# facebook/facebook360_dep

Measured on AMD Instinct MI355X. Metric: depth Mpix/s per GPU (full pyramid, 16-cam 2048^2 rig); % HBM-read roofline, higher is better.
Workload: dtype f32+f64; 1 GPU; BASELINE config 3: 16-camera 2048x2048 synthetic rig, 8-frame sequence, full 10-level pyramid per frame, per-level temporal filter (+-2 frames); the same sequence for every --gpus N (block partition, 8 frame(s) on this rank); rig=cfg2, cameras=16, frames=8, temporal_filter=True, halo_transport=local, parallelism=frames x1

## Files before the change

facebook360_dep_amd/csrc/derp_capi.hip:

```cpp
#include <hip/hip_runtime.h>

#include <algorithm>
#include <cfloat>
#include <cmath>
#include <cstdarg>
#include <cstdio>
#include <cstdlib>
#include <cstring>
#include <map>
#include <memory>
#include <string>
#include <vector>

#include <rocprim/device/device_radix_sort.hpp>

#include "../../include/derp_hip.h"
#include "derp_host.h"
#include "derp_kernels.h"
#include "derp_mesh.h"
#include "derp_points.h"
#include "derp_render.h"
#include "derp_geometric.h"
#include "derp_sweep.h"

// ... 360 lines not shown
  return 0;
}

int build_warp(derp_ctx* c, int dst0, int nd) {
  const int L = c->cur;
  Span sp(c, ST_PROJ_WARP, L);
  {
    const size_t n = (size_t)c->LW[L] * c->LH[L];
    ALLOC(c, c->rayDir, 3 * n * c->D * sizeof(double));
    ALLOC(c, c->behind, n * c->D * sizeof(unsigned));
  }
  LevelView V = make_view(c, ST_PROJ_WARP, dst0, nd);
  hipLaunchKernelGGL(k_proj_warp, grid2d(V.W + 2 * kPadW, V.H + 2 * kPadW, c->S, kBlk2d), kBlk2d, 0, c->stream, V,
                     c->projWarp.as<float2>());
  KCHECK(c);
  hipLaunchKernelGGL(k_pixel_rays, grid2d(V.W, V.H, nd, kBlk2d), kBlk2d, 0, c->stream, V, c->rayDir.as<double>(),
                     c->behind.as<unsigned>());
  KCHECK(c);
  c->w.colorTablesCleanLevel = -1;
  if (batch_needs_inverse_warps(c, dst0, nd)) {
    hipLaunchKernelGGL(k_proj_warp_inv, grid2d(V.W, V.H, nd, kBlk2d), kBlk2d, 0, c->stream, V, c->projWarpInv.as<float2>());
    KCHECK(c);
  }
  return 0;
}

int build_color_tables(derp_ctx* c, int dst0, int nd) {
  const int L = c->cur;
  LevelView V = make_view(c, ST_REPROJECT, dst0, nd);
  Span sp(c, ST_REPROJECT, L);
  const dim3 grid((V.W + kRbTile - 1) / kRbTile, (V.H + kRbTile - 1) / kRbTile, nd * (c->S - 1));
  ALLOC(c, c->w.tileSeen, (size_t)grid.x * grid.y * grid.z);
  const int skipBlank = c->w.colorTablesCleanLevel == L && nd == c->D && !c->noBlankSkip;
  hipLaunchKernelGGL(k_reproject_bias, grid, dim3(256), 0, c->stream, V, c->projWarpInv.as<float2>(),
                     c->w.projColor.as<ushort4>(), c->w.projBias.as<ushort4>(), c->w.projColorT.as<ushort4>(),
                     c->w.tileSeen.as<uint8_t>(), skipBlank);
  KCHECK(c);
  c->w.colorTablesCleanLevel = nd == c->D ? L : -1;
  return 0;
}

int tiles_of(int W, int H, int& tilesX) {
  constexpr int B = kTileBlock;
  tilesX = ((W + 15) / 16 + B - 1) / B * B;
  const int tilesY = ((H + 15) / 16 + B - 1) / B * B;
  return tilesX * tilesY * (256 / kCostBlock);
}
constexpr size_t kCostLdsPerSrc = (size_t)kCostBlock * sizeof(SsdPair);
struct CostGrid {
  int blocks, bands, perBlock;
};
constexpr int kCostMaxBands = 4, kCostMaxTilesPerBlock = 4;
int cost_grid_blocks(int tiles, int bands, int perBlock) {
  const int items = (tiles + perBlock - 1) / perBlock, unit = 8 * bands;
  return (items + unit - 1) / unit * unit;
}
CostGrid cost_grid(const derp_ctx* c, int tiles, int tilesX, bool spread) {
  const auto pow2_floor = [](int v, int cap) {
    int p = 1;
    while (p * 2 <= std::min(v, cap)) {
      p *= 2;
    }
    return p;
  };
  CostGrid g;
  g.perBlock = c->costTilesPerBlock > 0 ? pow2_floor(c->costTilesPerBlock, kCostMaxTilesPerBlock) : 1;
  const int rowOfSquares = tilesX * (256 / kCostBlock) * kTileBlock;
// ... 117 lines not shown
  }
  for (int d = 0; d < c->D; ++d) {
    if (c->dst2srcH[d] != d) {
      return fail(c, "mismatch handling needs destinations in rig order (dst %d maps to src %d)", d, c->dst2srcH[d]);
    }
  }
  Span sp(c, ST_MISMATCH, L);
  c->randomRanThisLevel = false;
  LevelView V = make_view(c, ST_MISMATCH, 0, c->D);
  const size_t n = (size_t)V.W * V.H;
  hipLaunchKernelGGL(k_mismatch, dim3((V.W + 15) / 16, (V.H + 15) / 16, c->D), dim3(256), 256 * sizeof(float) * c->S,
                     c->stream, V, c->w.dispRes.as<float>(), c->w.mismatchMask.as<uint8_t>());
  KCHECK(c);
  HIPCHK(c, hipMemcpyAsync(c->w.disparity.p, c->w.dispRes.p, n * c->D * sizeof(float), hipMemcpyDeviceToDevice, c->stream));
  return 0;
}

int bilateral_radius(int level) {
  const float scale = std::pow(0.9f, level);
  return (int)std::max(std::ceil(5 * scale), float(1));
}

size_t bilateral_lds_bytes(int radius) {
  const size_t side = 16 + 2 * (size_t)radius;
  const size_t t = ((side + 15) & ~(size_t)15) * side;
  return t * 4 * sizeof(float) + ((t + 3) & ~(size_t)3);
}

constexpr size_t kBilateralMaxLds = 64 * 1024 - 256;

bool bilateral_fast_tap_ok(float sigma, float w0, float w1, float w2) {
  const float denom = 2.0f * (sigma * sigma);
  return w1 == 1.0f && w2 == 1.0f && w0 >= 0.0f && std::isfinite(w0) && denom > 0.0f && std::isfinite(denom);
}

void launch_joint_bilateral_u16_tiled(derp_ctx* c, dim3 grid, const float* image, const void* guide, const uint8_t* mask,
                                      int W, int H, int radius, float sigma, float w0, float w1, float w2, float* out,
                                      size_t planeStride, size_t guideStride, const int* guideIndex) {
  const bool fast = bilateral_fast_tap_ok(sigma, w0, w1, w2) && bilateral_lds_bytes(radius) + 256 <= kBilateralMaxLds;
  const auto kernel = fast ? k_joint_bilateral<true, true> : k_joint_bilateral<true, false>;
  hipLaunchKernelGGL(kernel, grid, dim3(256), bilateral_lds_bytes(radius), c->stream, image, guide, mask, W, H, radius, sigma,
                     w0, w1, w2, out, planeStride, guideStride, guideIndex);
}

int run_bilateral(derp_ctx* c) {
  const int L = c->cur;
  Span sp(c, ST_BILATERAL, L);
  c->randomRanThisLevel = false;
  const int W = c->LW[L], H = c->LH[L];
  const size_t n = (size_t)W * H;
  const int radius = bilateral_radius(L);
  launch_joint_bilateral_u16_tiled(c, dim3((W + 15) / 16, (H + 15) / 16, c->D), c->w.disparity.as<float>(),
                                   (const void*)c->frame().color[L].as<ushort4>(), c->w.maskAnd.as<uint8_t>(), W, H, radius,
                                   0.005f, 0.5f, 1.0f, 1.0f, c->w.tmpF.as<float>(), n, n, c->dst2src.as<int>());
  KCHECK(c);
  std::swap(c->w.disparity, c->w.tmpF);
  return 0;
}

int run_median(derp_ctx* c, bool fuseMaskFov, float* levelOut = nullptr) {
  const int L = c->cur;
  Span sp(c, ST_MEDIAN, L);
  c->randomRanThisLevel = false;
  const int W = c->LW[L], H = c->LH[L];
  const size_t n = (size_t)W * H;
  hipLaunchKernelGGL(k_masked_median, grid2d(W, H, c->D, kBlk2d), kBlk2d, 0, c->stream, c->w.disparity.as<float>(),
// ... 281 lines not shown
    rc = fail(c, "work lane: hipEventRecord failed");
  }
  lane_swap(c, i);
  c->activeLane = -1;
  c->cur = -1;
  return rc;
}

int temporal_launch(derp_ctx* c, const void* const* guides, const float* const* images, const uint8_t* const* masks, int n,
                    int centre, int W, int H, int planes, float sigma, int radius, float w0, float w1, float w2,
                    float* out, const int* dst2src) {
  if (n < 1 || centre < 0 || centre >= n) {
    return fail(c, "temporal window must hold at least the centre frame");
  }
  if (n > kMaxTemporalFrames) {
    ALLOC(c, c->temporalCarry, (size_t)planes * W * H * sizeof(float2));
  }
  for (int t0 = 0; t0 < n; t0 += kMaxTemporalFrames) {
    TemporalFrames F;
    F.n = std::min(kMaxTemporalFrames, n - t0);
    for (int t = 0; t < F.n; ++t) {
      F.guides[t] = reinterpret_cast<const ushort4*>(guides[t0 + t]);
      F.images[t] = images[t0 + t];
      F.masks[t] = masks[t0 + t];
    }
    F.refGuide = reinterpret_cast<const ushort4*>(guides[centre]);
    F.refImage = images[centre];
    F.refMask = masks[centre];
    F.carry = n > kMaxTemporalFrames ? c->temporalCarry.as<float2>() : nullptr;
    F.first = t0 == 0;
    F.last = t0 + F.n >= n;
    const size_t lds = 2 * ((((size_t)(32 + 2 * radius) * (8 + 2 * radius) * 9) + 15) & ~(size_t)15);
    if (radius >= 0 && lds <= 48 * 1024 && !c->noTemporalTile) {
      hipLaunchKernelGGL(k_temporal_tiled, grid2d(W, H, planes, kBlk2d), kBlk2d, lds, c->stream, F, W, H, sigma, radius, w0,
                         w1, w2, out, dst2src);
    } else {
      hipLaunchKernelGGL(k_temporal, grid2d(W, H, planes, kBlk2d), kBlk2d, 0, c->stream, F, W, H, sigma, radius, w0, w1, w2,
                         out, dst2src);
    }
    KCHECK(c);
  }
  return 0;
}

}

extern "C" {

void derp_options_default(derp_options* o) {
  o->min_depth_m = 0.5f;
  o->max_depth_m = 1e4f;
  o->var_noise_floor = 4e-5f;
  o->var_high_thresh = 1e-3f;
  o->random_proposals = 2;
  o->ping_pong_iterations = 1;
  o->mismatches_start_level = -1;
  o->do_bilateral_filter = 1;
  o->do_median_filter = 1;
  o->use_foreground_masks = 0;
  o->partial_coverage = 0;
  o->rebuild_warp_tables = 1;
}

int derp_create(derp_ctx** out, int device, const derp_camera_desc* src, int n_src, const derp_camera_desc* dst,
                int n_dst) {
  if (!out) {
    return 1;
  }
// ... 4 lines not shown
  if (n_src <= 0 || n_dst <= 0) {
    return create_fail("no source / destination cameras!");
  }
  hipDeviceProp_t prop;
  TRY(open_device(device, "the depth path", &prop));
  c->device = device;
  if (prop.maxSharedMemoryPerMultiProcessor > 0) {
    c->ldsPerCu = prop.maxSharedMemoryPerMultiProcessor;
  }
  if (const char* e = getenv("DERP_XCD_ROTATE")) {
    c->xcdRotate = atoi(e);
  }
  if (const char* e = getenv("DERP_XCD_BANDS")) {
    c->xcdBands = atoi(e);
  }
  if (const char* e = getenv("DERP_COST_TILES_PER_BLOCK")) {
    c->costTilesPerBlock = atoi(e);
  }
  c->noMemo = getenv("DERP_NO_MEMO") != nullptr;
  if (const char* e = getenv("DERP_BRUTE_RUN")) {
    c->bruteRun = atoi(e);
  }
  if (const char* e = getenv("DERP_PP_COMPACT")) {
    c->ppCompact = atoi(e) != 0;
  }
  if (const char* e = getenv("DERP_RANDOM_WAVES")) {
    c->randomWaves = atoi(e);
  }
  if (const char* e = getenv("DERP_PP_WAVES")) {
    c->ppWaves = atoi(e);
  }
  c->noTemporalTile = getenv("DERP_NO_TEMPORAL_TILE") != nullptr;
  c->noBlankSkip = getenv("DERP_NO_BLANK_SKIP") != nullptr;
  c->S = n_src;
  c->D = n_dst;
  c->frames.resize(1);
  c->camsSrcH.resize(n_src);
  c->camsDstH.resize(n_dst);
  for (int i = 0; i < n_src; ++i) {
    if (const char* m = host_prepare_camera(src[i], c->camsSrcH[i])) {
      return create_fail(std::string("camera ") + src[i].id + ": " + m);
    }
  }
  c->dst2srcH.assign(n_dst, 0);
  c->descDstH.assign(dst, dst + n_dst);
  for (int i = 0; i < n_dst; ++i) {
    if (const char* m = host_prepare_camera(dst[i], c->camsDstH[i])) {
      return create_fail(std::string("camera ") + dst[i].id + ": " + m);
    }
    bool found = false;
    for (int s = 0; s < n_src; ++s) {
      if (strncmp(dst[i].id, src[s].id, sizeof dst[i].id) == 0) {
        c->dst2srcH[i] = s;
        found = true;
        break;
      }
    }
    if (!found) {
      return create_fail(std::string("destination camera ") + dst[i].id + " is not a source camera");
    }
    if (memcmp(&c->camsDstH[i], &c->camsSrcH[c->dst2srcH[i]], sizeof(Cam)) != 0) {
      return create_fail(std::string("destination camera ") + dst[i].id + " differs from the source camera of the same id "
                  "(destinations must be cameras of the source rig, as filterDestinations makes them)");
    }
  }
  if (c->camsSrc.ensure(sizeof(Cam) * n_src) || c->camsDst.ensure(sizeof(Cam) * n_dst) ||
// ... 442 lines not shown
```

facebook360_dep_amd/csrc/derp_ctx.h:

```cpp
#pragma once

namespace {

enum Stage {
  ST_FOV = 0,
  ST_VARIANCE,
  ST_OWN_BIAS,
  ST_UPSAMPLE,
  ST_PROJ_WARP,
  ST_REPROJECT,
  ST_PROJ_BIAS,
  ST_BRUTE,
  ST_RANDOM,
  ST_PINGPONG,
  ST_MISMATCH,
  ST_BILATERAL,
  ST_MEDIAN,
  ST_MASKFOV,
  ST_TEMPORAL,
  ST_LANES,
  ST_GC_PREPARE,
  ST_GC_SWEEP,
  ST_GC_CLEAN,
  ST_SWEEP_OVERLAPS,
// ... 79 lines not shown
  WorkSet w;
  DevBuf temporalCarry;
  DevBuf projWarp, projWarpInv;
  DevBuf rayDir, behind;
  int warpCachedLevel = -1;
  DevBuf fovMask;
  int fovCachedLevel = -1;
  bool randomRanThisLevel = false;
  bool tablesValid = false;
  std::map<std::pair<int, int>, LanczosTab> lanczos;
  std::map<std::pair<int, int>, AreaTabDev> areaTabs;
  DevBuf spiral;
  int spiralN = 0, spiralRadius = -1;
  std::vector<std::unique_ptr<WorkLane>> lanes;
  hipEvent_t laneReady = nullptr;
  int activeLane = -1;

  DevBuf counters;
  bool profiling = false;
  std::vector<TimedSpan> spans;
  double accMs[ST_COUNT][kMaxLevels] = {};
  int accLaunch[ST_COUNT][kMaxLevels] = {};
  int xcdRotate = 1;
  int xcdBands = 0, costTilesPerBlock = 0;
  DevBuf blockTrace[2][kMaxLevels];
  int blockTraceGrid[2][kMaxLevels][2] = {};
  bool noMemo = false;
  int bruteRun = 10;
  bool ppCompact = true;
  int randomWaves = 0, ppWaves = 0;
  size_t ldsPerCu = 160 * 1024;
  bool noTemporalTile = false;
  bool noBlankSkip = false;
  std::unique_ptr<SmrState> smr;
  std::unique_ptr<RephotoState> rephoto;
  std::unique_ptr<PointsState> points;
  std::unique_ptr<MeshState> mesh;
  std::unique_ptr<GcState> gc;
  std::unique_ptr<SweepState> sweep;
};

namespace {

int fail(derp_ctx* c, const char* fmt, ...) {
  va_list ap;
  va_start(ap, fmt);
  vfail(c ? &c->err : nullptr, fmt, ap);
  va_end(ap);
  return 1;
}

int use_device(derp_ctx* c) {
  if (!c) {
    return 1;
  }
  HIPCHK(c, hipSetDevice(c->device));
  return 0;
}

int check_camera(derp_ctx* c, int cam) {
  if (cam < 0 || cam >= c->D) {
    return fail(c, "bad camera index %d (the context has %d)", cam, c->D);
  }
  return 0;
}

// ... 2 lines not shown
```

facebook360_dep_amd/csrc/derp_debug_api.h:

```cpp
#pragma once

namespace {
struct HostPairs {
  SsdPair* p;
  SsdPair get(int i) const {
    return p[i];
  }
  void set(int i, const SsdPair& v) {
    p[i] = v;
  }
};
int stage_index(const char* stage) {
  for (int i = 0; i < ST_COUNT; ++i) {
    if (strcmp(stage, kStageNames[i]) == 0) {
      return i;
    }
  }
  return -1;
}
}

int derp_debug_atan2_ypos(derp_ctx* c, const double* y, const double* x, double* out, size_t n) {
  if (!c || !y || !x || !out) {
    return fail(c, "bad arguments");
// ... 76 lines not shown
    return 0;
  }
  if (d < 0 || d >= c->D || s < 0 || s >= c->S || s == c->dst2srcH[d]) {
    return fail(c, "bad (dst, src) pair");
  }
  const size_t tab = (size_t)d * (c->S - 1) + (s < c->dst2srcH[d] ? s : s - 1);
  if (which == 0) {
    const int PW = W + 2 * kPadW, PH = H + 2 * kPadW;
    std::vector<float2> tmp((size_t)PW * PH);
    HIPCHK(c, hipMemcpy(tmp.data(), c->projWarp.as<float2>() + tab * tmp.size(), tmp.size() * sizeof(float2),
                        hipMemcpyDeviceToHost));
    float2* o = reinterpret_cast<float2*>(out);
    for (int y = 0; y < H; ++y) {
      memcpy(o + (size_t)y * W, &tmp[(size_t)(y + kPadW) * PW + kPadW], (size_t)W * sizeof(float2));
    }
    return 0;
  }
  if (which == 2 || which == 3) {
    const int PW = W + 2 * kPadC, PH = H + 2 * kPadC;
    std::vector<ushort4> tmp((size_t)PW * PH);
    const ushort4* base = (which == 2 ? c->w.projColor.as<ushort4>() : c->w.projBias.as<ushort4>()) + tab * tmp.size();
    HIPCHK(c, hipMemcpy(tmp.data(), base, tmp.size() * sizeof(ushort4), hipMemcpyDeviceToHost));
    uint16_t* o = reinterpret_cast<uint16_t*>(out);
    for (int y = 0; y < H; ++y) {
      for (int x = 0; x < W; ++x) {
        const ushort4 q = tmp[(size_t)(y + kPadC) * PW + x + kPadC];
        o[((size_t)y * W + x) * 3 + 0] = q.x;
        o[((size_t)y * W + x) * 3 + 1] = q.y;
        o[((size_t)y * W + x) * 3 + 2] = q.z;
      }
    }
    return 0;
  }
  return fail(c, "unknown table id %d", which);
}

int derp_dev_disparity(derp_ctx* c, int level, int d, float** ptr, size_t* bytes) {
  TRY(check_level(c, level));
  if (d < 0 || d >= c->D || !ptr || !bytes) {
    return fail(c, "bad destination index / null output");
  }
  const size_t n = npx(c, level);
  *ptr = c->frame().disp[level].as<float>() + (size_t)d * n;
  *bytes = n * sizeof(float);
  return 0;
}
int derp_dev_color(derp_ctx* c, int level, int s, void** ptr, size_t* bytes) {
  TRY(check_level(c, level));
  if (s < 0 || s >= c->S || !ptr || !bytes) {
    return fail(c, "bad source index / null output");
  }
  const size_t n = npx(c, level);
  *ptr = c->frame().color[level].as<ushort4>() + (size_t)s * n;
  *bytes = n * sizeof(ushort4);
  return 0;
}
int derp_dev_mask(derp_ctx* c, int level, int d, uint8_t** ptr, size_t* bytes) {
  TRY(check_level(c, level));
  if (d < 0 || d >= c->D || !ptr || !bytes) {
    return fail(c, "bad destination index / null output");
  }
  HIPCHK(c, hipSetDevice(c->device));
  const int W = c->LW[level], H = c->LH[level];
  const size_t n = (size_t)W * H;
  ALLOC(c, c->devMask, n * c->D);
  hipLaunchKernelGGL(k_fov_mask, grid2d(W, H, c->D, kBlk2d), kBlk2d, 0, c->stream, c->camsDst.as<Cam>(), W, H,
// ... 191 lines not shown
```

facebook360_dep_amd/csrc/derp_kernels.h:

```cpp
#pragma once
#include <hip/hip_runtime.h>
#include <math.h>
#include <stdint.h>

#include <type_traits>

#include "derp_camera.h"
#include "gcc_algos.h"

namespace derp {

#ifndef DERP_COST_MIN_WAVES
#define DERP_COST_MIN_WAVES 4
#endif
#ifndef DERP_RANDOM_MIN_WAVES
#define DERP_RANDOM_MIN_WAVES 4
#endif
#ifndef DERP_RANDOM_TILED
#define DERP_RANDOM_TILED 0
#endif
#ifndef DERP_MIX_HOT_ONLY
#define DERP_MIX_HOT_ONLY 0
#endif
#ifndef DERP_PHASE_TIMERS
// ... 995 lines not shown
  const float nan = __builtin_nanf("");
  for (int dl = 0; dl < V.D; ++dl) {
    const int d = V.dst0 + dl;
    const int own = V.dst2src[d];
    if (s == own) {
      continue;
    }
    float2 val = make_float2(nan, nan);
    if (!outside) {
      const Cam& cd = V.camsDst[d];
      D2 p;
      if (sees(cd, rig, cd.principal[0] * W, cd.principal[1] * H, cd.focal[0] * W, cd.focal[1] * H, W, H, p)) {
        val = make_float2((float)(p.x - (double)0.5f), (float)(p.y - (double)0.5f));
      }
    }
    projWarp[((size_t)dl * (V.S - 1) + slot(s, own)) * plane + (size_t)oy * OW + ox] = val;
  }
}

__device__ __forceinline__ void cubic_coeffs(float x, float* c) {
  const float A = -0.75f;
  c[0] = ((A * (x + 1) - 5 * A) * (x + 1) + 8 * A) * (x + 1) - 4 * A;
  c[1] = ((A + 2) * x - (A + 3)) * x * x + 1;
  c[2] = ((A + 2) * (1 - x) - (A + 3)) * (1 - x) * (1 - x) + 1;
  c[3] = 1.f - c[0] - c[1] - c[2];
}
__device__ __forceinline__ int cv_round(float v) {
  if (!(v > -2147483648.0f && v < 2147483648.0f)) {
    return (int)0x80000000;
  }
  return (int)rintf(v);
}

__device__ __forceinline__ ushort4 remap_cubic_u16(const ushort4* __restrict__ img, int W, int H, float mx, float my) {
  const int fsx = cv_round(mx * 32.0f), fsy = cv_round(my * 32.0f);
  const int fx = fsx & 31, fy = fsy & 31;
  const int sx = min(max(fsx >> 5, -32768), 32767) - 1, sy = min(max(fsy >> 5, -32768), 32767) - 1;
  float cx[4], cy[4];
  cubic_coeffs((float)fx * (1.f / 32), cx);
  cubic_coeffs((float)fy * (1.f / 32), cy);
  float sum[3];
  if ((unsigned)sx < (unsigned)max(W - 3, 0) && (unsigned)sy < (unsigned)max(H - 3, 0)) {
    float rowsum[4][3];
#pragma unroll
    for (int i = 0; i < 4; ++i) {
      const u4a8* r = reinterpret_cast<const u4a8*>(img + (size_t)(sy + i) * W + sx);
      const u4a8 a = r[0], b = r[1];
      const float w0 = cy[i] * cx[0], w1 = cy[i] * cx[1], w2 = cy[i] * cx[2], w3 = cy[i] * cx[3];
      rowsum[i][0] = (float)(a.x & 0xffff) * w0 + (float)(a.z & 0xffff) * w1 + (float)(b.x & 0xffff) * w2 + (float)(b.z & 0xffff) * w3;
      rowsum[i][1] = (float)(a.x >> 16) * w0 + (float)(a.z >> 16) * w1 + (float)(b.x >> 16) * w2 + (float)(b.z >> 16) * w3;
      rowsum[i][2] = (float)(a.y & 0xffff) * w0 + (float)(a.w & 0xffff) * w1 + (float)(b.y & 0xffff) * w2 + (float)(b.w & 0xffff) * w3;
    }
#pragma unroll
    for (int c = 0; c < 3; ++c) {
      float acc = rowsum[0][c];
      acc += rowsum[1][c];
      acc += rowsum[2][c];
      acc += rowsum[3][c];
      sum[c] = acc;
    }
  } else if (sx >= W || sx + 4 <= 0 || sy >= H || sy + 4 <= 0) {
    sum[0] = sum[1] = sum[2] = 0.f;
  } else {
    sum[0] = sum[1] = sum[2] = 0.f;
    for (int i = 0; i < 4; ++i) {
      const int yy = sy + i;
      if ((unsigned)yy >= (unsigned)H) {
        continue;
      }
      for (int j = 0; j < 4; ++j) {
        const int xx = sx + j;
        if ((unsigned)xx >= (unsigned)W) {
          continue;
        }
        const ushort4 q = img[(size_t)yy * W + xx];
        const float w = cy[i] * cx[j];
        sum[0] += ((float)q.x - 0.f) * w;
        sum[1] += ((float)q.y - 0.f) * w;
        sum[2] += ((float)q.z - 0.f) * w;
      }
    }
  }
  const int r0 = min(max(cv_round(sum[0]), 0), 65535), r1 = min(max(cv_round(sum[1]), 0), 65535),
            r2 = min(max(cv_round(sum[2]), 0), 65535);
  return make_ushort4((unsigned short)r0, (unsigned short)r1, (unsigned short)r2, 0);
}

__device__ __forceinline__ int batch_dst_of_source(const LevelView& V, int s) {
  for (int dl = 0; dl < V.D; ++dl) {
    if (V.dst2src[V.dst0 + dl] == s) {
      return dl;
    }
  }
  return -1;
}

__device__ __forceinline__ bool dst_far_point(const LevelView& V, const Cam& cd, int x, int y, D3& rig) {
  const double W = V.W, H = V.H;
  const double dprx = cd.principal[0] * W, dpry = cd.principal[1] * H, dfx = cd.focal[0] * W, dfy = cd.focal[1] * H;
  const double px = x + 0.5, py = y + 0.5;
  if (outside_image_circle(cd, px, py, dprx, dpry, dfx, dfy)) {
    return false;
  }
  const D3 dir = rig_direction(cd, px, py, dprx, dpry, dfx, dfy);
  rig = {cd.pos[0] + dir.x * 1e4, cd.pos[1] + dir.y * 1e4, cd.pos[2] + dir.z * 1e4};
  return true;
}
__device__ __forceinline__ float2 warp_inv_of(const LevelView& V, const Cam& cs, bool inside, const D3& rig) {
  const double W = V.W, H = V.H;
  D2 p;
  if (inside && sees(cs, rig, cs.principal[0] * W, cs.principal[1] * H, cs.focal[0] * W, cs.focal[1] * H, W, H, p)) {
    return make_float2((float)(p.x - (double)0.5f), (float)(p.y - (double)0.5f));
  }
  const float nan = __builtin_nanf("");
  return make_float2(nan, nan);
}

__global__ void k_proj_warp_inv(LevelView V, float2* __restrict__ warpInv) {
// ... 63 lines not shown
  if (x >= V.W) {
    return;
  }
  const int oxa = x == 0 ? 0 : x + kPadC, oxb = x == V.W - 1 ? OW - 1 : x + kPadC;
#pragma unroll
  for (int j = 0; j < kRbTile / 8; ++j) {
    const int ly = (int)(threadIdx.x >> 5) + 8 * j;
    const int y = y0 + ly;
    if (y >= V.H) {
      break;
    }
    const ushort4* t = &tile[(ly + 1) * kRbPitch + lx + 1];
    unsigned s0 = 0, s1 = 0, s2 = 0;
#pragma unroll
    for (int v = -1; v <= 1; ++v) {
#pragma unroll
      for (int u = -1; u <= 1; ++u) {
        const ushort4 q = t[v * kRbPitch + u];
        s0 += q.x;
        s1 += q.y;
        s2 += q.z;
      }
    }
    const ushort4 col = t[0];
    const ushort4 bia = make_ushort4((unsigned short)((s0 + 4) / 9), (unsigned short)((s1 + 4) / 9),
                                     (unsigned short)((s2 + 4) / 9), 0);
    const int oya = y == 0 ? 0 : y + kPadC, oyb = y == V.H - 1 ? OH - 1 : y + kPadC;
    for (int oy = oya; oy <= oyb; ++oy) {
      for (int ox = oxa; ox <= oxb; ++ox) {
        pc[(size_t)oy * OW + ox] = col;
        pb[(size_t)oy * OW + ox] = bia;
        if (pt) {
          pt[tiled_index(tilesX, ox, oy)] = col;
        }
      }
    }
  }
}

__device__ __forceinline__ float probe_disparity(int i, float minD, float maxD) {
  const double fraction = (double)i / (double)(kNumDepths - 1);
  return (float)(fraction * (double)minD + (1 - fraction) * (double)maxD);
}

__global__ void __launch_bounds__(kCostBlock, DERP_COST_MIN_WAVES)
    k_brute_costs(LevelView V, float* __restrict__ costs, float* __restrict__ confs, int tilesX, int tilesPerDst, int run) {
  const int i0 = blockIdx.y * run, i1 = min(i0 + run, kNumDepths);
  const int dl = blockIdx.z;
  const int d = V.dst0 + dl;
  const int iw = V.W - 2, ih = V.H - 2;
  const int lane = threadIdx.x & 63;
  const int sx = (int)(blockIdx.x % (unsigned)tilesX), sy = (int)(blockIdx.x / (unsigned)tilesX);
  const int x = 1 + sx * 8 + (lane & 7), y = 1 + sy * 8 + (lane >> 3);
  PatchWin* win;
  LdsPairs pairs = cost_wave_prologue(V, d, x - (int)(threadIdx.x & 7), y - (int)((threadIdx.x & 63) >> 3), win);
  unsigned nCost = 0, nPair = 0;
  if (x <= iw && y <= ih) {
    const int own = V.dst2src[d];
    const size_t n = (size_t)V.W * V.H, idx = (size_t)y * V.W + x;
    const float minDisparity = 1.0f / V.maxDepthM, maxDisparity = 1.0f / V.minDepthM;
    const bool fov = V.fovMask[(size_t)d * n + idx], fg = V.srcFg[(size_t)own * n + idx];
    const float nan = __builtin_nanf("");
    if (fov && fg) {
      PixCtx px;
      load_pixctx<false>(V, d, own, x, y, win, px);
      const unsigned cull = behind_sources(V, d, idx);
// ... 1374 lines not shown
    weightedSumPix = acc.x;
    sumWeight = acc.y;
  }
  for (int t = 0; t < F.n; ++t) {
    const float centre = F.images[t][pd + idx];
    const uint8_t* __restrict__ mask = F.masks[t] + pd;
    const ushort4* __restrict__ guide = F.guides[t] + pg;
    for (int u = -radius; u <= radius; ++u) {
      const int sx = min(max(x + u, 0), W - 1);
      for (int v = -radius; v <= radius; ++v) {
        const int sy = min(max(y + v, 0), H - 1);
        const size_t j = (size_t)sy * W + sx;
        if (!mask[j]) {
          continue;
        }
        const ushort4 sc = guide[j];
        const float e0 = div_int_by_const((int)ref.x - (int)sc.x, rcp65535);
        const float e1 = div_int_by_const((int)ref.y - (int)sc.y, rcp65535);
        const float e2 = div_int_by_const((int)ref.z - (int)sc.z, rcp65535);
        const float weightedDiff = weight0 * (e0 * e0) + weight1 * (e1 * e1) + weight2 * (e2 * e2);
        const float weight = expf_glibc(div_by_const(-weightedDiff, rcpSig2), expTab);
        weightedSumPix += centre * weight;
        sumWeight += weight;
      }
    }
  }
  if (F.last) {
    out[pd + idx] = weightedSumPix / sumWeight;
  } else {
    F.carry[pd + idx] = make_float2(weightedSumPix, sumWeight);
  }
}

__global__ void __launch_bounds__(256)
    k_temporal_tiled(TemporalFrames F, int W, int H, float sigma, int radius, float weight0, float weight1, float weight2,
                     float* __restrict__ out, const int* __restrict__ dst2src) {
  extern __shared__ unsigned char ldsTemporal[];
  __shared__ unsigned long long expTab[32];
  const int tid = threadIdx.y * blockDim.x + threadIdx.x;
  if (tid < 32) {
    expTab[tid] = kExp2fTab[tid];
  }
  const int TW = 32 + 2 * radius, TH = 8 + 2 * radius, cells = TW * TH;
  const size_t bufBytes = ((size_t)cells * 9 + 15) & ~(size_t)15;
  const int x0 = blockIdx.x * 32, y0 = blockIdx.y * 8;
  const int x = x0 + threadIdx.x, y = y0 + threadIdx.y;
  const bool inside = x < W && y < H;
  const size_t n = (size_t)W * H;
  const size_t pd = (size_t)blockIdx.z * n, pg = dst2src ? (size_t)dst2src[blockIdx.z] * n : 0;
  const size_t idx = inside ? (size_t)y * W + x : 0;
  const bool active = inside && F.refMask[pd + idx] != 0;
  ushort4 ref = make_ushort4(0, 0, 0, 0);
  float weightedSumPix = 0.f, sumWeight = 0.f;
  if (active) {
    ref = F.refGuide[pg + idx];
    if (!F.first) {
      const float2 acc = F.carry[pd + idx];
      weightedSumPix = acc.x;
      sumWeight = acc.y;
    }
  }
  const float sig2 = sigma * sigma;
  const double rcpSig2 = 1.0 / (double)sig2;
  const double rcp65535 = 1.0 / 65535.0;
  int cellSrc[2];
#pragma unroll
  for (int i = 0; i < 2; ++i) {
    const int k = min(tid + i * 256, cells - 1);
    const int ty = k / TW, tx = k - ty * TW;
    const int sx = min(max(x0 - radius + tx, 0), W - 1), sy = min(max(y0 - radius + ty, 0), H - 1);
    cellSrc[i] = sy * W + sx;
  }
  ushort4 nextG[2];
  unsigned char nextM[2];
  float centreNext = 0.f;
  auto fetch = [&](int t) {
    const uint8_t* __restrict__ mask = F.masks[t] + pd;
    const ushort4* __restrict__ guide = F.guides[t] + pg;
#pragma unroll
    for (int i = 0; i < 2; ++i) {
      nextM[i] = mask[cellSrc[i]];
      nextG[i] = guide[cellSrc[i]];
    }
    if (active) {
      centreNext = F.images[t][pd + idx];
    }
  };
  auto stash = [&](int t) {
    unsigned char* buf = ldsTemporal + (size_t)(t & 1) * bufBytes;
    ushort4* tg = reinterpret_cast<ushort4*>(buf);
    unsigned char* tm = buf + (size_t)cells * 8;
#pragma unroll
    for (int i = 0; i < 2; ++i) {
      const int k = tid + i * 256;
      if (k < cells) {
        tm[k] = nextM[i];
        tg[k] = nextG[i];
      }
    }
    if (cells > 512) {
      const uint8_t* __restrict__ mask = F.masks[t] + pd;
      const ushort4* __restrict__ guide = F.guides[t] + pg;
      for (int k = tid + 512; k < cells; k += 256) {
        const int ty = k / TW, tx = k - ty * TW;
        const int sx = min(max(x0 - radius + tx, 0), W - 1), sy = min(max(y0 - radius + ty, 0), H - 1);
        const size_t j = (size_t)sy * W + sx;
        tm[k] = mask[j];
        tg[k] = guide[j];
      }
    }
  };
  fetch(0);
  stash(0);
  for (int t = 0; t < F.n; ++t) {
    const unsigned char* buf = ldsTemporal + (size_t)(t & 1) * bufBytes;
    const ushort4* tg = reinterpret_cast<const ushort4*>(buf);
    const unsigned char* tm = buf + (size_t)cells * 8;
    const float centre = centreNext;
    __syncthreads();
    if (t + 1 < F.n) {
      fetch(t + 1);
    }
    if (active) {
      for (int u = -radius; u <= radius; ++u) {
        for (int v = -radius; v <= radius; ++v) {
          const int k = ((int)threadIdx.y + radius + v) * TW + (int)threadIdx.x + radius + u;
          if (!tm[k]) {
            continue;
          }
          const ushort4 sc = tg[k];
          const float e0 = div_int_by_const((int)ref.x - (int)sc.x, rcp65535);
          const float e1 = div_int_by_const((int)ref.y - (int)sc.y, rcp65535);
          const float e2 = div_int_by_const((int)ref.z - (int)sc.z, rcp65535);
          const float weightedDiff = weight0 * (e0 * e0) + weight1 * (e1 * e1) + weight2 * (e2 * e2);
          const float weight = expf_glibc(div_by_const(-weightedDiff, rcpSig2), expTab);
          weightedSumPix += centre * weight;
          sumWeight += weight;
        }
      }
    }
    if (t + 1 < F.n) {
      stash(t + 1);
    }
  }
  if (!inside) {
    return;
  }
  if (!active) {
    if (F.last) {
      out[pd + idx] = F.refImage[pd + idx];
    }
    return;
  }
  if (F.last) {
    out[pd + idx] = weightedSumPix / sumWeight;
  } else {
    F.carry[pd + idx] = make_float2(weightedSumPix, sumWeight);
  }
}

__global__ void k_rephoto_splat(const Cam* __restrict__ cams, int target, const float* __restrict__ disps, int W, int H,
                                unsigned long long* __restrict__ key) {
  const int x = blockIdx.x * blockDim.x + threadIdx.x, y = blockIdx.y * blockDim.y + threadIdx.y;
  const int j = blockIdx.z;
  if (x >= W || y >= H || j == target) {
    return;
  }
  const size_t n = (size_t)W * H, idx = (size_t)y * W + x;
  const float d = disps[(size_t)j * n + idx];
  if (!(d > 0) || isinf(d)) {
// ... 435 lines not shown
```

facebook360_dep_amd/derp.py:

```python
import ctypes as C
import os

import numpy as np

_HERE = os.path.dirname(os.path.abspath(__file__))
LIB_PATH = os.environ.get("DERP_LIB") or os.path.join(_HERE, "libderp_hip.so")
CAM_TYPES = {"FTHETA": 0, "RECTILINEAR": 1, "EQUISOLID": 2, "ORTHOGRAPHIC": 3}

STAGES = ["fov_mask", "variance", "own_bias", "upsample", "proj_warp", "reproject", "proj_bias", "brute_force",
          "random_proposals", "ping_pong", "mismatches", "bilateral", "median", "mask_fov", "temporal"]


class SeqOptions(C.Structure):
    _fields_ = [
        ("time_radius", C.c_int32), ("sigma", C.c_float), ("weight_b", C.c_float), ("weight_g", C.c_float),
        ("weight_r", C.c_float), ("space_radius", C.c_int32), ("use_foreground_masks", C.c_int32),
        ("partition", C.c_int32), ("do_temporal_filter", C.c_int32), ("resident_frames", C.c_int32),
    ]


class SeqTransfer(C.Structure):
    _fields_ = [("frame", C.c_int32), ("from_rank", C.c_int32), ("to_rank", C.c_int32)]


# ... 365 lines not shown
    def debug_atan2_ypos(self, y, x):
        y = np.ascontiguousarray(y, np.float64)
        x = np.ascontiguousarray(x, np.float64)
        out = np.zeros_like(y)
        self._ck(lib().derp_debug_atan2_ypos(self.h, _p(y), _p(x), _p(out), C.c_size_t(y.size)))
        return out

    FP64_OPS = {"sqrt_lean": 0, "sqrt": 1, "div_plain": 2, "div": 3}

    def debug_fp64(self, op, a, b=None):
        a = np.ascontiguousarray(a, np.float64)
        b = None if b is None else np.ascontiguousarray(b, np.float64)
        assert b is None or b.shape == a.shape
        out = np.zeros_like(a)
        self._ck(lib().derp_debug_fp64(self.h, self.FP64_OPS[op], _p(a), _p(b), _p(out), C.c_size_t(a.size)))
        return out

    def debug_expf(self, x, nonpos=False):
        x = np.ascontiguousarray(x, np.float32)
        out = np.zeros_like(x)
        self._ck(lib().derp_debug_expf(self.h, int(bool(nonpos)), _p(x), _p(out), C.c_size_t(x.size)))
        return out

    def debug_sees(self, src, xyz):
        xyz = np.ascontiguousarray(xyz, np.float64).reshape(-1, 3)
        out = np.zeros((len(xyz), 2, 3))
        self._ck(lib().derp_debug_sees(self.h, src, _p(xyz), C.c_size_t(len(xyz)), _p(out)))
        return out[:, :, 0].T != 0, np.ascontiguousarray(out[:, :, 1:].transpose(1, 0, 2))

    def debug(self, d, s, which):
        h, w = self._shape(self._cur)
        spec = {"warp": (0, (h, w, 2), np.float32), "color": (2, (h, w, 3), np.uint16),
                "bias": (3, (h, w, 3), np.uint16), "variance": (4, (h, w), np.float32),
                "fov": (5, (h, w), np.uint8)}[which]
        out = np.zeros(spec[1], dtype=spec[2])
        self._ck(lib().derp_debug_download(self.h, d, s, spec[0], _p(out)))
        return out

    def mismatch_mask(self, d):
        out = np.zeros(self._shape(self._cur), dtype=np.uint8)
        self._ck(lib().derp_download_mismatch_mask(self.h, d, _p(out)))
        return out

    def layer_disparities(self, fg, bg):
        fg = np.ascontiguousarray(fg, dtype=np.float32)
        bg = np.ascontiguousarray(bg, dtype=np.float32)
        out = np.zeros(fg.shape, dtype=np.uint8)
        self._ck(lib().derp_layer_disparities(self.h, _p(fg), _p(bg), C.c_size_t(fg.size), _p(out)))
        return out

    def ssim(self, x, y, blur_radius=1, alpha=1.0, beta=1.0, gamma=1.0):
        x = np.ascontiguousarray(x, dtype=np.float32)
        y = np.ascontiguousarray(y, dtype=np.float32)
        h, w = x.shape[:2]
        out = np.zeros((h, w, 3), dtype=np.float32)
        self._ck(lib().derp_ssim(self.h, _p(x), _p(y), w, h, blur_radius, C.c_float(alpha), C.c_float(beta),
                                 C.c_float(gamma), _p(out)))
        return out

    def rephotograph(self, target, colors, disps):
        colors = [np.ascontiguousarray(c, dtype=np.uint16) for c in colors]
        disps = [np.ascontiguousarray(d, dtype=np.float32) for d in disps]
        h, w = disps[0].shape
        cp = (C.c_void_p * len(colors))(*[c.ctypes.data for c in colors])
        dp = (C.c_void_p * len(disps))(*[d.ctypes.data for d in disps])
        out = np.zeros((h, w, 4), dtype=np.float32)
        self._ck(lib().derp_rephotograph(self.h, target, cp, dp, w, h, _p(out)))
# ... 743 lines not shown
```

Before: 513.2 Mpix/s.

## Add front-loaded reproject kernel and fast-path temporal filter specialisations

Adds a new reprojection kernel that precomputes a shared cubic coefficient table and classifies cells up front, so all interior bicubic taps are issued together with wave-uniform branching. It also specialises the tiled temporal filter on radius and a fast mode that skips per-tap mask checks when the whole staged tile is valid and uses a non-positive exp variant. Debug download modes for the padded colour tables and the tile-seen flags are added too. Env flags allow falling back to the old paths. The new kernels carry more code, add register pressure, and are a correctness risk at image borders.

```diff
diff --git a/facebook360_dep_amd/csrc/derp_capi.hip b/facebook360_dep_amd/csrc/derp_capi.hip
--- a/facebook360_dep_amd/csrc/derp_capi.hip
+++ b/facebook360_dep_amd/csrc/derp_capi.hip
@@ -416,7 +416,8 @@
   const dim3 grid((V.W + kRbTile - 1) / kRbTile, (V.H + kRbTile - 1) / kRbTile, nd * (c->S - 1));
   ALLOC(c, c->w.tileSeen, (size_t)grid.x * grid.y * grid.z);
   const int skipBlank = c->w.colorTablesCleanLevel == L && nd == c->D && !c->noBlankSkip;
-  hipLaunchKernelGGL(k_reproject_bias, grid, dim3(256), 0, c->stream, V, c->projWarpInv.as<float2>(),
+  const auto kernel = c->reprojectSerial ? k_reproject_bias : k_reproject_bias_front;
+  hipLaunchKernelGGL(kernel, grid, dim3(256), 0, c->stream, V, c->projWarpInv.as<float2>(),
                      c->w.projColor.as<ushort4>(), c->w.projBias.as<ushort4>(), c->w.projColorT.as<ushort4>(),
                      c->w.tileSeen.as<uint8_t>(), skipBlank);
   KCHECK(c);
@@ -600,6 +601,12 @@
 bool bilateral_fast_tap_ok(float sigma, float w0, float w1, float w2) {
   const float denom = 2.0f * (sigma * sigma);
   return w1 == 1.0f && w2 == 1.0f && w0 >= 0.0f && std::isfinite(w0) && denom > 0.0f && std::isfinite(denom);
+}
+
+bool temporal_fast_tap_ok(float sigma, float w0, float w1, float w2) {
+  const float sig2 = sigma * sigma;
+  const auto weight_ok = [](float w) { return w >= 0.0f && std::isfinite(w); };
+  return weight_ok(w0) && weight_ok(w1) && weight_ok(w2) && sig2 > 0.0f && std::isfinite(sig2);
 }
 
 void launch_joint_bilateral_u16_tiled(derp_ctx* c, dim3 grid, const float* image, const void* guide, const uint8_t* mask,
@@ -947,8 +954,10 @@
     F.last = t0 + F.n >= n;
     const size_t lds = 2 * ((((size_t)(32 + 2 * radius) * (8 + 2 * radius) * 9) + 15) & ~(size_t)15);
     if (radius >= 0 && lds <= 48 * 1024 && !c->noTemporalTile) {
-      hipLaunchKernelGGL(k_temporal_tiled, grid2d(W, H, planes, kBlk2d), kBlk2d, lds, c->stream, F, W, H, sigma, radius, w0,
-                         w1, w2, out, dst2src);
+      const bool fast = temporal_fast_tap_ok(sigma, w0, w1, w2) && !c->temporalGeneric;
+      const auto kernel = !fast ? k_temporal_tiled<-1, false> : radius == 1 ? k_temporal_tiled<1, true> : k_temporal_tiled<-1, true>;
+      hipLaunchKernelGGL(kernel, grid2d(W, H, planes, kBlk2d), kBlk2d, lds, c->stream, F, W, H, sigma, radius, w0, w1, w2, out,
+                         dst2src);
     } else {
       hipLaunchKernelGGL(k_temporal, grid2d(W, H, planes, kBlk2d), kBlk2d, 0, c->stream, F, W, H, sigma, radius, w0, w1, w2,
                          out, dst2src);
@@ -1019,6 +1028,12 @@
   }
   c->noTemporalTile = getenv("DERP_NO_TEMPORAL_TILE") != nullptr;
   c->noBlankSkip = getenv("DERP_NO_BLANK_SKIP") != nullptr;
+  if (const char* e = getenv("DERP_TEMPORAL_GENERIC")) {
+    c->temporalGeneric = atoi(e) != 0;
+  }
+  if (const char* e = getenv("DERP_REPROJECT_SERIAL")) {
+    c->reprojectSerial = atoi(e) != 0;
+  }
   c->S = n_src;
   c->D = n_dst;
   c->frames.resize(1);
diff --git a/facebook360_dep_amd/csrc/derp_ctx.h b/facebook360_dep_amd/csrc/derp_ctx.h
--- a/facebook360_dep_amd/csrc/derp_ctx.h
+++ b/facebook360_dep_amd/csrc/derp_ctx.h
@@ -135,6 +135,7 @@
   size_t ldsPerCu = 160 * 1024;
   bool noTemporalTile = false;
   bool noBlankSkip = false;
+  bool temporalGeneric = false, reprojectSerial = false;
   std::unique_ptr<SmrState> smr;
   std::unique_ptr<RephotoState> rephoto;
   std::unique_ptr<PointsState> points;
diff --git a/facebook360_dep_amd/csrc/derp_debug_api.h b/facebook360_dep_amd/csrc/derp_debug_api.h
--- a/facebook360_dep_amd/csrc/derp_debug_api.h
+++ b/facebook360_dep_amd/csrc/derp_debug_api.h
@@ -132,6 +132,23 @@
     }
     return 0;
   }
+  if (which == 6 || which == 7) {
+    const size_t plane = (size_t)(W + 2 * kPadC) * (H + 2 * kPadC);
+    const DevBuf& buf = which == 6 ? c->w.projColor : c->w.projBias;
+    if (buf.bytes < (tab + 1) * plane * sizeof(ushort4)) {
+      return fail(c, "the colour tables of this level have not been built");
+    }
+    HIPCHK(c, hipMemcpy(out, buf.as<ushort4>() + tab * plane, plane * sizeof(ushort4), hipMemcpyDeviceToHost));
+    return 0;
+  }
+  if (which == 8) {
+    const size_t tiles = (size_t)((W + kRbTile - 1) / kRbTile) * ((H + kRbTile - 1) / kRbTile);
+    if (c->w.tileSeen.bytes < (tab + 1) * tiles) {
+      return fail(c, "the colour tables of this level have not been built");
+    }
+    HIPCHK(c, hipMemcpy(out, c->w.tileSeen.as<uint8_t>() + tab * tiles, tiles, hipMemcpyDeviceToHost));
+    return 0;
+  }
   return fail(c, "unknown table id %d", which);
 }
 
diff --git a/facebook360_dep_amd/csrc/derp_kernels.h b/facebook360_dep_amd/csrc/derp_kernels.h
--- a/facebook360_dep_amd/csrc/derp_kernels.h
+++ b/facebook360_dep_amd/csrc/derp_kernels.h
@@ -1051,36 +1051,60 @@
   return (int)rintf(v);
 }
 
+struct CubicTaps {
+  u4a8 a[4], b[4];
+};
+__device__ __forceinline__ void cubic_rows_sum(const CubicTaps& t, const float* cx, const float* cy, float* sum) {
+  float rowsum[4][3];
+#pragma unroll
+  for (int i = 0; i < 4; ++i) {
+    const u4a8 a = t.a[i], b = t.b[i];
+    const float w0 = cy[i] * cx[0], w1 = cy[i] * cx[1], w2 = cy[i] * cx[2], w3 = cy[i] * cx[3];
+    rowsum[i][0] = (float)(a.x & 0xffff) * w0 + (float)(a.z & 0xffff) * w1 + (float)(b.x & 0xffff) * w2 + (float)(b.z & 0xffff) * w3;
+    rowsum[i][1] = (float)(a.x >> 16) * w0 + (float)(a.z >> 16) * w1 + (float)(b.x >> 16) * w2 + (float)(b.z >> 16) * w3;
+    rowsum[i][2] = (float)(a.y & 0xffff) * w0 + (float)(a.w & 0xffff) * w1 + (float)(b.y & 0xffff) * w2 + (float)(b.w & 0xffff) * w3;
+  }
+#pragma unroll
+  for (int c = 0; c < 3; ++c) {
+    float acc = rowsum[0][c];
+    acc += rowsum[1][c];
+    acc += rowsum[2][c];
+    acc += rowsum[3][c];
+    sum[c] = acc;
+  }
+}
+__device__ __forceinline__ void cubic_interior_sum(const CubicTaps& t, int fx, int fy, float* sum) {
+  float cx[4], cy[4];
+  cubic_coeffs((float)fx * (1.f / 32), cx);
+  cubic_coeffs((float)fy * (1.f / 32), cy);
+  cubic_rows_sum(t, cx, cy, sum);
+}
+__device__ __forceinline__ ushort4 cubic_saturate_u16(const float* sum) {
+  const int r0 = min(max(cv_round(sum[0]), 0), 65535), r1 = min(max(cv_round(sum[1]), 0), 65535),
+            r2 = min(max(cv_round(sum[2]), 0), 65535);
+  return make_ushort4((unsigned short)r0, (unsigned short)r1, (unsigned short)r2, 0);
+}
+
 __device__ __forceinline__ ushort4 remap_cubic_u16(const ushort4* __restrict__ img, int W, int H, float mx, float my) {
   const int fsx = cv_round(mx * 32.0f), fsy = cv_round(my * 32.0f);
   const int fx = fsx & 31, fy = fsy & 31;
   const int sx = min(max(fsx >> 5, -32768), 32767) - 1, sy = min(max(fsy >> 5, -32768), 32767) - 1;
-  float cx[4], cy[4];
-  cubic_coeffs((float)fx * (1.f / 32), cx);
-  cubic_coeffs((float)fy * (1.f / 32), cy);
   float sum[3];
   if ((unsigned)sx < (unsigned)max(W - 3, 0) && (unsigned)sy < (unsigned)max(H - 3, 0)) {
-    float rowsum[4][3];
+    CubicTaps t;
 #pragma unroll
     for (int i = 0; i < 4; ++i) {
       const u4a8* r = reinterpret_cast<const u4a8*>(img + (size_t)(sy + i) * W + sx);
-      const u4a8 a = r[0], b = r[1];
-      const float w0 = cy[i] * cx[0], w1 = cy[i] * cx[1], w2 = cy[i] * cx[2], w3 = cy[i] * cx[3];
-      rowsum[i][0] = (float)(a.x & 0xffff) * w0 + (float)(a.z & 0xffff) * w1 + (float)(b.x & 0xffff) * w2 + (float)(b.z & 0xffff) * w3;
-      rowsum[i][1] = (float)(a.x >> 16) * w0 + (float)(a.z >> 16) * w1 + (float)(b.x >> 16) * w2 + (float)(b.z >> 16) * w3;
-      rowsum[i][2] = (float)(a.y & 0xffff) * w0 + (float)(a.w & 0xffff) * w1 + (float)(b.y & 0xffff) * w2 + (float)(b.w & 0xffff) * w3;
-    }
-#pragma unroll
-    for (int c = 0; c < 3; ++c) {
-      float acc = rowsum[0][c];
-      acc += rowsum[1][c];
-      acc += rowsum[2][c];
-      acc += rowsum[3][c];
-      sum[c] = acc;
-    }
+      t.a[i] = r[0];
+      t.b[i] = r[1];
+    }
+    cubic_interior_sum(t, fx, fy, sum);
   } else if (sx >= W || sx + 4 <= 0 || sy >= H || sy + 4 <= 0) {
     sum[0] = sum[1] = sum[2] = 0.f;
   } else {
+    float cx[4], cy[4];
+    cubic_coeffs((float)fx * (1.f / 32), cx);
+    cubic_coeffs((float)fy * (1.f / 32), cy);
     sum[0] = sum[1] = sum[2] = 0.f;
     for (int i = 0; i < 4; ++i) {
       const int yy = sy + i;
@@ -1100,9 +1124,7 @@
       }
     }
   }
-  const int r0 = min(max(cv_round(sum[0]), 0), 65535), r1 = min(max(cv_round(sum[1]), 0), 65535),
-            r2 = min(max(cv_round(sum[2]), 0), 65535);
-  return make_ushort4((unsigned short)r0, (unsigned short)r1, (unsigned short)r2, 0);
+  return cubic_saturate_u16(sum);
 }
 
 __device__ __forceinline__ int batch_dst_of_source(const LevelView& V, int s) {
@@ -1232,6 +1254,178 @@
         pb[(size_t)oy * OW + ox] = bia;
         if (pt) {
           pt[tiled_index(tilesX, ox, oy)] = col;
+        }
+      }
+    }
+  }
+}
+
+__device__ __forceinline__ int reflect101_near(int p, int len) {
+  return len == 1 ? 0 : p < 0 ? -p : p >= len ? 2 * len - 2 - p : p;
+}
+enum : unsigned {
+  kRbZero = 0,
+  kRbInterior = 1,
+  kRbBorder = 2,
+  kRbNone = 3
+};
+constexpr int kRbTrips = (kRbCells + 255) / 256;
+
+__global__ void __launch_bounds__(256, 6)
+    k_reproject_bias_front(LevelView V, const float2* __restrict__ warpInv, ushort4* __restrict__ projColor,
+                           ushort4* __restrict__ projBias, ushort4* __restrict__ projColorT, uint8_t* __restrict__ tileSeen,
+                           int skipBlank) {
+  __shared__ ushort4 tile[kRbCells];
+  __shared__ float4 coefTab[32];
+  const int tab = blockIdx.z;
+  uint8_t* seen = tileSeen + ((size_t)tab * gridDim.y + blockIdx.y) * gridDim.x + blockIdx.x;
+  if (skipBlank && !*seen) {
+    return;
+  }
+  if (threadIdx.x < 32) {
+    float c[4];
+    cubic_coeffs((float)(int)threadIdx.x * (1.f / 32), c);
+    coefTab[threadIdx.x] = make_float4(c[0], c[1], c[2], c[3]);
+  }
+  const int dl = tab / (V.S - 1), sl = tab - dl * (V.S - 1);
+  const int own = V.dst2src[V.dst0 + dl];
+  const int s = sl < own ? sl : sl + 1;
+  const int x0 = blockIdx.x * kRbTile, y0 = blockIdx.y * kRbTile;
+  const int W = V.W, H = V.H;
+  const int OW = W + 2 * kPadC, OH = H + 2 * kPadC;
+  const size_t plane = (size_t)OW * OH, n = (size_t)W * H;
+  const ushort4* img = V.srcColor + (size_t)s * n;
+  const float2* map = warpInv + (size_t)tab * n;
+  int mapPitch = W;
+  const int ds = batch_dst_of_source(V, s);
+  if (ds >= 0) {
+    mapPitch = W + 2 * kPadW;
+    map = V.projWarp + ((size_t)ds * (V.S - 1) + slot(own, s)) * warp_plane(V) + (size_t)kPadW * mapPitch + kPadW;
+  }
+  const int tid = threadIdx.x;
+  float2 m[kRbTrips];
+  bool cell[kRbTrips];
+  {
+    int ty = tid / kRbPitch, tx = tid - ty * kRbPitch;
+#pragma unroll
+    for (int i = 0; i < kRbTrips; ++i) {
+      const int qx = x0 - 1 + tx, qy = y0 - 1 + ty;
+      cell[i] = tid + 256 * i < kRbCells && qx <= W && qy <= H;
+      const int rx = reflect101_near(min(qx, W), W), ry = reflect101_near(min(qy, H), H);
+      m[i] = at32(map, (unsigned)(ry * mapPitch + rx));
+      tx += 256 % kRbPitch;
+      ty += 256 / kRbPitch;
+      if (tx >= kRbPitch) {
+        tx -= kRbPitch;
+        ++ty;
+      }
+    }
+  }
+  unsigned off[kRbTrips], st[kRbTrips];
+  int any = 0;
+#pragma unroll
+  for (int i = 0; i < kRbTrips; ++i) {
+    const int fsx = cv_round(m[i].x * 32.0f), fsy = cv_round(m[i].y * 32.0f);
+    const int sx = min(max(fsx >> 5, -32768), 32767) - 1, sy = min(max(fsy >> 5, -32768), 32767) - 1;
+    const bool valid = cell[i] && !(m[i].x != m[i].x);
+    any |= valid;
+    const bool interior = valid && (unsigned)sx < (unsigned)max(W - 3, 0) && (unsigned)sy < (unsigned)max(H - 3, 0);
+    const bool outside = sx >= W || sx + 4 <= 0 || sy >= H || sy + 4 <= 0;
+    const unsigned kind = !cell[i] ? kRbNone : interior ? kRbInterior : (!valid || outside) ? kRbZero : kRbBorder;
+    off[i] = interior ? (unsigned)(sy * W + sx) * 8u : 0u;
+    st[i] = (unsigned)(fsx & 31) | (unsigned)(fsy & 31) << 5 | kind << 10;
+  }
+  __syncthreads();
+  const unsigned rowBytes = (unsigned)W * 8u;
+  const char* imgB = reinterpret_cast<const char*>(img);
+#pragma unroll
+  for (int i = 0; i < kRbTrips; ++i) {
+    const unsigned kind = st[i] >> 10;
+    ushort4 res = make_ushort4(0, 0, 0, 0);
+    if (__ballot(kind == kRbInterior) != 0) {
+      CubicTaps t;
+#pragma unroll
+      for (int r = 0; r < 4; ++r) {
+        t.a[r] = *reinterpret_cast<const u4a8*>(imgB + (off[i] + (unsigned)r * rowBytes));
+        t.b[r] = *reinterpret_cast<const u4a8*>(imgB + (off[i] + (unsigned)r * rowBytes + 16u));
+      }
+      const float4 tx4 = coefTab[st[i] & 31], ty4 = coefTab[st[i] >> 5 & 31];
+      const float cx[4] = {tx4.x, tx4.y, tx4.z, tx4.w}, cy[4] = {ty4.x, ty4.y, ty4.z, ty4.w};
+      float sum[3];
+      cubic_rows_sum(t, cx, cy, sum);
+      const ushort4 r = cubic_saturate_u16(sum);
+      if (kind == kRbInterior) {
+        res = r;
+      }
+    }
+    if (__ballot(kind == kRbBorder) != 0) {
+      if (kind == kRbBorder) {
+        const int k = tid + 256 * i;
+        const int ty = k / kRbPitch, tx = k - ty * kRbPitch;
+        const int rx = reflect101_near(x0 - 1 + tx, W), ry = reflect101_near(y0 - 1 + ty, H);
+        const float2 mb = at32(map, (unsigned)(ry * mapPitch + rx));
+        res = remap_cubic_u16(img, W, H, mb.x, mb.y);
+      }
+    }
+    if (kind != kRbNone) {
+      tile[tid + 256 * i] = res;
+    }
+  }
+  any = __syncthreads_or(any);
+  if (!skipBlank && threadIdx.x == 0) {
+    *seen = (uint8_t)(any != 0);
+  }
+  ushort4* pc = projColor + (size_t)tab * plane;
+  ushort4* pb = projBias + (size_t)tab * plane;
+  const int tilesX = tiled_tiles_x(W);
+  ushort4* pt = projColorT ? projColorT + (size_t)tab * tiled_plane(W, H) : nullptr;
+  const int lx = tid & 31;
+  const int x = x0 + lx;
+  if (x >= W) {
+    return;
+  }
+  const bool edge = x0 == 0 || y0 == 0 || x0 + kRbTile >= W || y0 + kRbTile >= H;
+  const int oxa = x == 0 ? 0 : x + kPadC, oxb = x == W - 1 ? OW - 1 : x + kPadC;
+#pragma unroll
+  for (int j = 0; j < kRbTile / 8; ++j) {
+    const int ly = (tid >> 5) + 8 * j;
+    const int y = y0 + ly;
+    if (y >= H) {
+      break;
+    }
+    const ushort4* t = &tile[(ly + 1) * kRbPitch + lx + 1];
+    unsigned s0 = 0, s1 = 0, s2 = 0;
+#pragma unroll
+    for (int v = -1; v <= 1; ++v) {
+#pragma unroll
+      for (int u = -1; u <= 1; ++u) {
+        const ushort4 q = t[v * kRbPitch + u];
+        s0 += q.x;
+        s1 += q.y;
+        s2 += q.z;
+      }
+    }
+    const ushort4 col = t[0];
+    const float ninth = 1.0f / 9.0f;
+    const ushort4 bia = make_ushort4((unsigned short)(int)((float)(s0 + 4) * ninth), (unsigned short)(int)((float)(s1 + 4) * ninth),
+                                     (unsigned short)(int)((float)(s2 + 4) * ninth), 0);
+    if (!edge) {
+      const unsigned o = (unsigned)((y + kPadC) * OW + x + kPadC);
+      at32(pc, o) = col;
+      at32(pb, o) = bia;
+      if (pt) {
+        at32(pt, (unsigned)tiled_index(tilesX, x + kPadC, y + kPadC)) = col;
+      }
+      continue;
+    }
+    const int oya = y == 0 ? 0 : y + kPadC, oyb = y == H - 1 ? OH - 1 : y + kPadC;
+    for (int oy = oya; oy <= oyb; ++oy) {
+      for (int ox = oxa; ox <= oxb; ++ox) {
+        const unsigned o = (unsigned)(oy * OW + ox);
+        at32(pc, o) = col;
+        at32(pb, o) = bia;
+        if (pt) {
+          at32(pt, (unsigned)tiled_index(tilesX, ox, oy)) = col;
         }
       }
     }
@@ -2672,15 +2866,32 @@
   }
 }
 
+template <bool FAST>
+__device__ __forceinline__ void temporal_tap(ushort4 ref, ushort4 sc, float centre, float weight0, float weight1,
+                                             float weight2, double rcpSig2, const unsigned long long* expTab,
+                                             float& weightedSumPix, float& sumWeight) {
+  const double rcp65535 = 1.0 / 65535.0;
+  const float e0 = div_int_by_const((int)ref.x - (int)sc.x, rcp65535);
+  const float e1 = div_int_by_const((int)ref.y - (int)sc.y, rcp65535);
+  const float e2 = div_int_by_const((int)ref.z - (int)sc.z, rcp65535);
+  const float weightedDiff = weight0 * (e0 * e0) + weight1 * (e1 * e1) + weight2 * (e2 * e2);
+  const float arg = div_by_const(-weightedDiff, rcpSig2);
+  const float weight = FAST ? expf_glibc_nonpos(arg, expTab) : expf_glibc(arg, expTab);
+  weightedSumPix += centre * weight;
+  sumWeight += weight;
+}
+
+template <int RADIUS, bool FAST>
 __global__ void __launch_bounds__(256)
-    k_temporal_tiled(TemporalFrames F, int W, int H, float sigma, int radius, float weight0, float weight1, float weight2,
-                     float* __restrict__ out, const int* __restrict__ dst2src) {
+    k_temporal_tiled(TemporalFrames F, int W, int H, float sigma, int radiusArg, float weight0, float weight1,
+                     float weight2, float* __restrict__ out, const int* __restrict__ dst2src) {
   extern __shared__ unsigned char ldsTemporal[];
   __shared__ unsigned long long expTab[32];
   const int tid = threadIdx.y * blockDim.x + threadIdx.x;
   if (tid < 32) {
     expTab[tid] = kExp2fTab[tid];
   }
+  const int radius = RADIUS >= 0 ? RADIUS : radiusArg;
   const int TW = 32 + 2 * radius, TH = 8 + 2 * radius, cells = TW * TH;
   const size_t bufBytes = ((size_t)cells * 9 + 15) & ~(size_t)15;
   const int x0 = blockIdx.x * 32, y0 = blockIdx.y * 8;
@@ -2702,7 +2913,6 @@
   }
   const float sig2 = sigma * sigma;
   const double rcpSig2 = 1.0 / (double)sig2;
-  const double rcp65535 = 1.0 / 65535.0;
   int cellSrc[2];
 #pragma unroll
   for (int i = 0; i < 2; ++i) {
@@ -2714,6 +2924,7 @@
   ushort4 nextG[2];
   unsigned char nextM[2];
   float centreNext = 0.f;
+  int stagedFull = 1;
   auto fetch = [&](int t) {
     const uint8_t* __restrict__ mask = F.masks[t] + pd;
     const ushort4* __restrict__ guide = F.guides[t] + pg;
@@ -2730,10 +2941,12 @@
     unsigned char* buf = ldsTemporal + (size_t)(t & 1) * bufBytes;
     ushort4* tg = reinterpret_cast<ushort4*>(buf);
     unsigned char* tm = buf + (size_t)cells * 8;
+    stagedFull = 1;
 #pragma unroll
     for (int i = 0; i < 2; ++i) {
       const int k = tid + i * 256;
       if (k < cells) {
+        stagedFull &= nextM[i] != 0;
         tm[k] = nextM[i];
         tg[k] = nextG[i];
       }
@@ -2745,7 +2958,9 @@
         const int ty = k / TW, tx = k - ty * TW;
         const int sx = min(max(x0 - radius + tx, 0), W - 1), sy = min(max(y0 - radius + ty, 0), H - 1);
         const size_t j = (size_t)sy * W + sx;
-        tm[k] = mask[j];
+        const unsigned char mk = mask[j];
+        stagedFull &= mk != 0;
+        tm[k] = mk;
         tg[k] = guide[j];
       }
     }
@@ -2757,25 +2972,44 @@
     const ushort4* tg = reinterpret_cast<const ushort4*>(buf);
     const unsigned char* tm = buf + (size_t)cells * 8;
     const float centre = centreNext;
-    __syncthreads();
+    bool fullMask = false;
+    if (FAST) {
+      fullMask = __syncthreads_and(stagedFull) != 0;
+    } else {
+      __syncthreads();
+    }
     if (t + 1 < F.n) {
       fetch(t + 1);
     }
     if (active) {
-      for (int u = -radius; u <= radius; ++u) {
-        for (int v = -radius; v <= radius; ++v) {
-          const int k = ((int)threadIdx.y + radius + v) * TW + (int)threadIdx.x + radius + u;
-          if (!tm[k]) {
-            continue;
+      if (FAST && fullMask) {
+        if (RADIUS == 1) {
+          const ushort4* tc = tg + ((int)threadIdx.y + 1) * (32 + 2) + (int)threadIdx.x + 1;
+#pragma unroll
+          for (int u = -1; u <= 1; ++u) {
+#pragma unroll
+            for (int v = -1; v <= 1; ++v) {
+              temporal_tap<true>(ref, tc[v * (32 + 2) + u], centre, weight0, weight1, weight2, rcpSig2, expTab,
+                                 weightedSumPix, sumWeight);
+            }
           }
-          const ushort4 sc = tg[k];
-          const float e0 = div_int_by_const((int)ref.x - (int)sc.x, rcp65535);
-          const float e1 = div_int_by_const((int)ref.y - (int)sc.y, rcp65535);
-          const float e2 = div_int_by_const((int)ref.z - (int)sc.z, rcp65535);
-          const float weightedDiff = weight0 * (e0 * e0) + weight1 * (e1 * e1) + weight2 * (e2 * e2);
-          const float weight = expf_glibc(div_by_const(-weightedDiff, rcpSig2), expTab);
-          weightedSumPix += centre * weight;
-          sumWeight += weight;
+        } else {
+          for (int u = -radius; u <= radius; ++u) {
+            for (int v = -radius; v <= radius; ++v) {
+              const int k = ((int)threadIdx.y + radius + v) * TW + (int)threadIdx.x + radius + u;
+              temporal_tap<true>(ref, tg[k], centre, weight0, weight1, weight2, rcpSig2, expTab, weightedSumPix, sumWeight);
+            }
+          }
+        }
+      } else {
+        for (int u = -radius; u <= radius; ++u) {
+          for (int v = -radius; v <= radius; ++v) {
+            const int k = ((int)threadIdx.y + radius + v) * TW + (int)threadIdx.x + radius + u;
+            if (!tm[k]) {
+              continue;
+            }
+            temporal_tap<FAST>(ref, tg[k], centre, weight0, weight1, weight2, rcpSig2, expTab, weightedSumPix, sumWeight);
+          }
         }
       }
     }
diff --git a/facebook360_dep_amd/derp.py b/facebook360_dep_amd/derp.py
--- a/facebook360_dep_amd/derp.py
+++ b/facebook360_dep_amd/derp.py
@@ -421,7 +421,9 @@
         h, w = self._shape(self._cur)
         spec = {"warp": (0, (h, w, 2), np.float32), "color": (2, (h, w, 3), np.uint16),
                 "bias": (3, (h, w, 3), np.uint16), "variance": (4, (h, w), np.float32),
-                "fov": (5, (h, w), np.uint8)}[which]
+                "fov": (5, (h, w), np.uint8),
+                "color_padded": (6, (h + 4, w + 4, 4), np.uint16), "bias_padded": (7, (h + 4, w + 4, 4), np.uint16),
+                "tile_seen": (8, ((h + 31) // 32, (w + 31) // 32), np.uint8)}[which]
         out = np.zeros(spec[1], dtype=spec[2])
         self._ck(lib().derp_debug_download(self.h, d, s, spec[0], _p(out)))
         return out
```

Result: faster. 521.2 Mpix/s (median of 6 runs) (+1.6%).
